# boqian-li/GarmentDreamer

Hardware: AMD Instinct MI355X
Metric: SDS iters/sec (rasterize+UNet+bwd), 100k Gaussians ×8 views @512², 1/2/4/8 GPU (higher is better)
Workload: dtype bf16

## Files before the change

garmentdreamer_amd/csrc/nn_conv3x3.hip:

```cpp
#include <hip/hip_runtime.h>
#include <stdlib.h>
#include <stdint.h>
#include <stdio.h>

#include <mutex>
#include <vector>

#include "../../include/gd_nn.h"
#include "nn_device.h"
#include "nn_host.h"

#ifndef GD_CONV_ABLATE
#define GD_CONV_ABLATE 0
#endif

namespace {

using namespace gdnn;

#ifndef GD_PATCH_EPI
#define GD_PATCH_EPI 0
#endif
typedef __attribute__((ext_vector_type(4))) float f32x4;

constexpr int BK = 64;

struct ConvGeom {
    int Hin, Win, Hg, Wg, sy, sx, Hout, Wout, osy, osx, ooy, oox, ntaps, back;
    int wtaps;
    uint64_t ty4, tx4, w4;
};

template <int BN, int BM, int WN, int WM>
__device__ __forceinline__ void conv3x3_nhwc_bf16_body(
    const uint16_t* __restrict__ in, const uint16_t* __restrict__ wt, const uint16_t* __restrict__ bias,
    int bias_img_stride, const uint16_t* __restrict__ residual, uint16_t* __restrict__ out, int Nimg, const ConvGeom& g,
    int Cin, int Cout, int tiles_n, int nwg, float* __restrict__ partial, int steps_per_split, int bid_raw, int split_idx)
{
    constexpr int THREADS = 64 * WN * WM;
    constexpr int NA = BM * 8 / THREADS;
    constexpr int NB = BN * 8 / THREADS;
    constexpr int FA = BN / WN / 32;
    constexpr int FB = BM / WM / 32;
    constexpr int kStage = (BM + BN) * BK * 2;
    extern __shared__ __attribute__((aligned(16))) char smem[];
    const int tid = threadIdx.x, lane = tid & 63;
    const int wave = __builtin_amdgcn_readfirstlane(tid >> 6);
    int bid = bid_raw;
    if ((nwg & 7) == 0) bid = (bid & 7) * (nwg >> 3) + (bid >> 3);
    const int tn = bid % tiles_n, tm = bid / tiles_n;
    const int m0 = tm * BM, n0 = tn * BN;
    const int HW = g.Hg * g.Wg;
    const int64_t M = (int64_t)Nimg * HW;
    const int H = g.Hin, W = g.Win;

    const uint32_t row_bytes = (uint32_t)Cin * 2u;
    const uint32_t back = (uint32_t)g.back * row_bytes;
    const __amdgpu_buffer_rsrc_t rs_in = buffer_rsrc((const char*)in - back, (uint32_t)Nimg * (uint32_t)(H * W) * row_bytes + back);
    const __amdgpu_buffer_rsrc_t rs_w = buffer_rsrc(wt, (uint32_t)Cout * (uint32_t)g.wtaps * row_bytes);

    uint32_t a_off[NA];
    int a_y[NA], a_x[NA];
    uint32_t b_off[NB];
#pragma unroll
    for (int i = 0; i < NA; i++) {
        const int q = tid + THREADS * i;
        const int line = q >> 4, c = (q & 15) ^ (line & 15);
        const int r = 2 * line + (c >> 3);
        const int64_t m = (int64_t)m0 + r;
        if (m < M) {
            const int nimg = (int)(m / HW);
            const int rem = (int)(m - (int64_t)nimg * HW);
            const int ga = rem / g.Wg;
            a_y[i] = ga * g.sy;
            a_x[i] = (rem - ga * g.Wg) * g.sx;
            a_off[i] = (uint32_t)((nimg * H + a_y[i]) * W + a_x[i]) * row_bytes + (uint32_t)(c & 7) * 16u;
        } else {
            a_y[i] = -100000; a_x[i] = 0; a_off[i] = kOOB;
        }
    }
#pragma unroll
    for (int i = 0; i < NB; i++) {
        const int q = tid + THREADS * i;
        const int line = q >> 4, c = (q & 15) ^ (line & 15);
        const int r = 2 * line + (c >> 3);
        const int co = n0 + r;
        b_off[i] = co < Cout ? (uint32_t)co * (uint32_t)g.wtaps * row_bytes + (uint32_t)(c & 7) * 16u : kOOB;
    }
    const int kc = Cin / BK;
    const int step0 = partial ? split_idx * steps_per_split : 0;
    const int step1 = partial ? min(g.ntaps * kc, step0 + steps_per_split) : g.ntaps * kc;
    const int nsteps = step1 - step0;
    const int tap0 = step0 / kc;

    int ld_tap = tap0, ld_c = step0 - tap0 * kc;
    uint32_t a_voff[NA];
    auto set_tap = [&](int tap) {
        const int dy = (int)((g.ty4 >> (4 * tap)) & 15u) - 8, dx = (int)((g.tx4 >> (4 * tap)) & 15u) - 8;
#pragma unroll
        for (int i = 0; i < NA; i++) {
            const int yy = a_y[i] + dy, xx = a_x[i] + dx;
            const bool ok = (unsigned)yy < (unsigned)H && (unsigned)xx < (unsigned)W;
            a_voff[i] = ok ? a_off[i] : kOOB;
        }
    };
    set_tap(tap0);
    auto issue = [&](int buf) {
        char* sA = smem + buf * kStage;
        char* sB = sA + BM * BK * 2;
        const int dy = (int)((g.ty4 >> (4 * ld_tap)) & 15u) - 8, dx = (int)((g.tx4 >> (4 * ld_tap)) & 15u) - 8;
        const uint32_t soff_a = (uint32_t)(dy * W + dx + g.back) * row_bytes + (uint32_t)ld_c * (BK * 2);
        const uint32_t soff_b = (uint32_t)((g.w4 >> (4 * ld_tap)) & 15u) * row_bytes + (uint32_t)ld_c * (BK * 2);
#if GD_CONV_ABLATE != 1 && GD_CONV_ABLATE != 2 && GD_CONV_ABLATE < 6
#pragma unroll
        for (int i = 0; i < NA; i++) bload_lds16(rs_in, a_voff[i], soff_a, sA + (wave * 64 + THREADS * i) * 16);
#endif
#if GD_CONV_ABLATE != 2 && GD_CONV_ABLATE < 6
#pragma unroll
        for (int i = 0; i < NB; i++) bload_lds16(rs_w, b_off[i], soff_b, sB + (wave * 64 + THREADS * i) * 16);
#endif
        if (++ld_c == kc) {
            ld_c = 0;
            if (++ld_tap < g.ntaps) set_tap(ld_tap);
        }
    };

    f32x16 acc[FA][FB];
#pragma unroll
    for (int a = 0; a < FA; a++)
#pragma unroll
        for (int b = 0; b < FB; b++)
#pragma unroll
            for (int k = 0; k < 16; k++) acc[a][b][k] = 0.f;

    const int wc = wave % WN, wp = wave / WN;
    const int frow = lane & 31, fk = lane >> 5;
    uint32_t w_rd[FA], p_rd[FB];
#pragma unroll
    for (int a = 0; a < FA; a++) w_rd[a] = (uint32_t)(BM * BK * 2 + swz(wc * (BN / WN) + a * 32 + frow, fk));
#pragma unroll
    for (int b = 0; b < FB; b++) p_rd[b] = (uint32_t)swz(wp * (BM / WM) + b * 32 + frow, fk);

#if GD_CONV_ABLATE == 4 || GD_CONV_ABLATE >= 6
    bf16x8_t wf0[FA], pf0[FB];
#pragma unroll
    for (int a = 0; a < FA; a++) wf0[a] = *(const bf16x8_t*)(smem + w_rd[a]);
#pragma unroll
    for (int b = 0; b < FB; b++) pf0[b] = *(const bf16x8_t*)(smem + p_rd[b]);
#endif
    issue(0);
#if GD_CONV_ABLATE == 8
    for (int s = 0; s < (nsteps > 1 ? 1 : nsteps); s++) {
#else
    for (int s = 0; s < nsteps; s++) {
#endif
        const int buf = s & 1;
        asm volatile("s_waitcnt vmcnt(0)" ::: "memory");
#if GD_CONV_ABLATE != 5 && GD_CONV_ABLATE != 6
        __syncthreads();
#endif
        if (s + 1 < nsteps) issue(buf ^ 1);
        const char* st = smem + buf * kStage;
#pragma unroll
        for (int kk = 0; kk < 4; kk++) {
            bf16x8_t wf[FA], pf[FB];
#if GD_CONV_ABLATE == 4 || GD_CONV_ABLATE >= 6
            if (s > 0) {
#pragma unroll
                for (int a = 0; a < FA; a++)
#pragma unroll
                    for (int b = 0; b < FB; b++)
                        acc[a][b] = __builtin_amdgcn_mfma_f32_32x32x16_bf16(wf0[a], pf0[b], acc[a][b], 0, 0, 0);
                continue;
            }
#endif
#pragma unroll
            for (int a = 0; a < FA; a++) wf[a] = *(const bf16x8_t*)(st + (w_rd[a] ^ (uint32_t)(kk << 5)));
#pragma unroll
            for (int b = 0; b < FB; b++) pf[b] = *(const bf16x8_t*)(st + (p_rd[b] ^ (uint32_t)(kk << 5)));
#pragma unroll
            for (int a = 0; a < FA; a++)
#pragma unroll
                for (int b = 0; b < FB; b++)
#if GD_CONV_ABLATE == 3
                    if (a == 0 && b == 0) acc[a][b] = __builtin_amdgcn_mfma_f32_32x32x16_bf16(wf[a], pf[b], acc[a][b], 0, 0, 0);
                    else { acc[a][b][0] += __builtin_bit_cast(float, (int)wf[a][0] ^ (int)pf[b][1]); }
#else
                    acc[a][b] = __builtin_amdgcn_mfma_f32_32x32x16_bf16(wf[a], pf[b], acc[a][b], 0, 0, 0);
#endif
        }
    }

#pragma unroll
    for (int b = 0; b < FB; b++) {
        const int64_t m = (int64_t)m0 + wp * (BM / WM) + b * 32 + (lane & 31);
        if (m >= M) continue;
        const int nimg = (int)(m / HW);
// ... 4 lines not shown
#pragma unroll
        for (int a = 0; a < FA; a++) {
#pragma unroll
            for (int q = 0; q < 4; q++) {
                const int co = n0 + wc * (BN / WN) + a * 32 + 8 * q + 4 * fk;
                if (co >= Cout) continue;
                float v[4];
#pragma unroll
                for (int e = 0; e < 4; e++) v[e] = acc[a][b][4 * q + e];
                if (partial) {
                    *(float4*)(partial + (((size_t)split_idx * nwg + bid) * (BN * BM / 4) +
                                          (((wave * FB + b) * FA + a) * 4 + q) * 64 + lane) * 4) = make_float4(v[0], v[1], v[2], v[3]);
                    continue;
                }
                if (bias_n) {
                    const uint2 bb = *(const uint2*)(bias_n + co);
                    v[0] += bf2f((uint16_t)(bb.x & 0xffff)); v[1] += bf2f((uint16_t)(bb.x >> 16));
                    v[2] += bf2f((uint16_t)(bb.y & 0xffff)); v[3] += bf2f((uint16_t)(bb.y >> 16));
                }
                if (residual) {
                    const uint2 rr = *(const uint2*)(residual + opix * Cout + co);
                    v[0] += bf2f((uint16_t)(rr.x & 0xffff)); v[1] += bf2f((uint16_t)(rr.x >> 16));
                    v[2] += bf2f((uint16_t)(rr.y & 0xffff)); v[3] += bf2f((uint16_t)(rr.y >> 16));
                }
                uint2 o;
                o.x = pack_bf16(v[0], v[1]);
                o.y = pack_bf16(v[2], v[3]);
                *(uint2*)(out + opix * Cout + co) = o;
            }
        }
    }
}

template <int BN, int BM, int WN, int WM>
__global__ __launch_bounds__(64 * WN * WM) void conv3x3_nhwc_bf16_kernel(
    const uint16_t* __restrict__ in, const uint16_t* __restrict__ wt, const uint16_t* __restrict__ bias,
    int bias_img_stride, const uint16_t* __restrict__ residual, uint16_t* __restrict__ out, int Nimg, const ConvGeom g,
    int Cin, int Cout, int tiles_n, int nwg, float* __restrict__ partial, int steps_per_split)
{
    conv3x3_nhwc_bf16_body<BN, BM, WN, WM>(in, wt, bias, bias_img_stride, residual, out, Nimg, g, Cin, Cout, tiles_n, nwg,
                                           partial, steps_per_split, (int)blockIdx.x, (int)blockIdx.y);
}

struct ConvGeomSet {
    ConvGeom g[4];
    const uint16_t* wt[4];
    int nwg[4];
    int n;
};

template <int BN, int BM, int WN, int WM>
__global__ __launch_bounds__(64 * WN * WM) void conv3x3_nhwc_bf16_multi_kernel(
    const uint16_t* __restrict__ in, const uint16_t* __restrict__ bias, int bias_img_stride,
    const uint16_t* __restrict__ residual, uint16_t* __restrict__ out, int Nimg, const ConvGeomSet gs, int Cin, int Cout,
    int tiles_n)
{
    const int cls = (int)blockIdx.z;
    const int nwg = gs.nwg[cls];
    if ((int)blockIdx.x >= nwg) return;
    conv3x3_nhwc_bf16_body<BN, BM, WN, WM>(in, gs.wt[cls], bias, bias_img_stride, residual, out, Nimg, gs.g[cls], Cin, Cout,
                                           tiles_n, nwg, nullptr, 0, (int)blockIdx.x, 0);
}

constexpr int kPatch = 18, kPatchPix = kPatch * kPatch;

__device__ __forceinline__ float silu_fast(float z) { return z * __builtin_amdgcn_rcpf(1.0f + __expf(-z)); }

__device__ __forceinline__ float row16_sum(float v)
{
    v += __builtin_bit_cast(float, __builtin_amdgcn_update_dpp(0, __builtin_bit_cast(int, v), 0xB1, 0xf, 0xf, false));
    v += __builtin_bit_cast(float, __builtin_amdgcn_update_dpp(0, __builtin_bit_cast(int, v), 0x4E, 0xf, 0xf, false));
    v += __builtin_bit_cast(float, __builtin_amdgcn_update_dpp(0, __builtin_bit_cast(int, v), 0x141, 0xf, 0xf, false));
    v += __builtin_bit_cast(float, __builtin_amdgcn_update_dpp(0, __builtin_bit_cast(int, v), 0x140, 0xf, 0xf, false));
    return v;
}

__device__ __forceinline__ void stat_accumulate(float2& st, uint2 o)
{
    const float r0 = __uint_as_float(o.x << 16), r1 = __uint_as_float(o.x & 0xffff0000u);
    const float r2 = __uint_as_float(o.y << 16), r3 = __uint_as_float(o.y & 0xffff0000u);
    st.x += (r0 + r1) + (r2 + r3);
    st.y += fmaf(r0, r0, fmaf(r1, r1, fmaf(r2, r2, r3 * r3)));
}

__device__ __forceinline__ void patch_col(int fn, int& rr, int& fx)
{
    if (fn < 4) { rr = 0; fx = fn; }
    else if (fn < 12) { rr = 1; fx = fn - 4; }
    else if (fn < 16) { rr = 0; fx = fn - 8; }
    else if (fn < 20) { rr = 1; fx = fn - 8; }
    else if (fn < 28) { rr = 0; fx = fn - 12; }
    else { rr = 1; fx = fn - 16; }
}
// ... 733 lines not shown
            }
        }
        if (stat_part) {
            const int rows = nwaves * 2, row = wave_g * 2 + ((lane >> 4) & 1);
#pragma unroll
            for (int a = 0; a < FA; a++) {
#pragma unroll
                for (int q = 0; q < 4; q++) {
                    const float sx = row16_sum(st[a][q].x), sy = row16_sum(st[a][q].y);
                    const int quad = 8 * a + 2 * q + fk;
                    if ((lane & 15) == 0)
                        *(float2*)(stat_part + (((size_t)n * (Cout >> 2) + quad) * rows + row) * 2) = make_float2(sx, sy);
                }
            }
        }
    }
}

__global__ void conv3x3_flip_weights_kernel(const uint16_t* __restrict__ w, uint16_t* __restrict__ wf, int Cout,
                                            int Cin)
{
    const size_t total = (size_t)Cout * 9 * Cin;
    for (size_t i = (size_t)blockIdx.x * blockDim.x + threadIdx.x; i < total; i += (size_t)gridDim.x * blockDim.x) {
        const int co = (int)(i % Cout);
        const int tap = (int)((i / Cout) % 9);
        const int ci = (int)(i / ((size_t)Cout * 9));
        wf[i] = w[((size_t)co * 9 + (8 - tap)) * Cin + ci];
    }
}

int g_route_scale = 1;
int g_force_split = -1;
int g_force_variant = -1;

struct ConvEnv {
    int split_px = 0;
    int multi_class = 1;
    int patch_persistent = 1;
    int first_grid = 2048;
};
const ConvEnv& conv_env()
{
    static const ConvEnv env = [] {
        ConvEnv v;
        if (const char* e = getenv("GD_NN_SPLIT_PX")) v.split_px = atoi(e);
        if (const char* e = getenv("GD_NN_CONV_MULTI")) v.multi_class = atoi(e);
        if (const char* e = getenv("GD_NN_PATCH_PERSISTENT")) v.patch_persistent = atoi(e) != 0;
        if (const char* e = getenv("GD_NN_FIRST_GRID")) v.first_grid = atoi(e) > 0 ? atoi(e) : v.first_grid;
        return v;
    }();
    return env;
}

int num_cus(int dev)
{
    static const int cus = [dev] {
        int c = 0;
        return hipDeviceGetAttribute(&c, hipDeviceAttributeMultiprocessorCount, dev) == hipSuccess && c > 0 ? c : 256;
    }();
    return cus;
}

struct ConvProf {
    std::mutex mu;
    bool on = false;
    struct Rec { hipEvent_t a, b; };
// ... 168 lines not shown
    if (!x || !weight || !y) return fail(GD_NN_ERR_INVALID_ARG, "null pointer");
    if (N <= 0 || H <= 0 || W <= 0 || Cin % BK || Cout % 4 || Cin <= 0 || Cout <= 0)
        return fail(GD_NN_ERR_INVALID_ARG, "conv3x3: need Cin % 64 == 0 and Cout % 4 == 0");
    g = ConvGeom{};
    g.Hin = g.Hg = g.Hout = H;
    g.Win = g.Wg = g.Wout = W;
    g.sy = g.sx = g.osy = g.osx = 1;
    for (int ky = 0; ky < 3; ky++)
        for (int kx = 0; kx < 3; kx++) add_tap(g, ky - 1, kx - 1, ky * 3 + kx);
    return GD_NN_OK;
}

static int launch_conv(hipStream_t s, const void* x, const void* weight, const void* bias, int bias_img_stride,
                       const void* residual, void* y, int N, ConvGeom g, int Cin, int Cout, void* ws = nullptr,
                       size_t ws_bytes = 0)
{
    const int dev = current_device();
    if (dev < 0) return dev;
    if (const int r = finalize_geom(g, N, Cin, Cout)) return r;
    const int64_t M = (int64_t)N * g.Hg * g.Wg;
    if (M <= 0) return GD_NN_OK;
    int split = ws ? choose_split(M, Cout, g.ntaps, Cin) : 1;
    if (split > 1 && ws_bytes < split_ws_bytes(split, M, Cout)) split = 1;
    float* partial = split > 1 ? (float*)ws : nullptr;
    const int total_steps = g.ntaps * (Cin / BK);
    const int tps = split > 1 ? (total_steps + split - 1) / split : total_steps;
    if (split > 1) split = (total_steps + tps - 1) / tps;
    const int spx = split > 1 ? split_tile_px(M, Cout) : 128;
    int variant = split > 1 ? (spx == 256 ? 1 : 0) : g_force_variant;
    if (variant < 0 && small_tile_nosplit(M, Cout, g.ntaps, Cin)) variant = 6;
    if (variant < 0)
        variant = Cout <= 32 && M * g_route_scale >= (1 << 18) ? 4 : tile_variant(M, Cin, Cout);
    ProfScope prof(s);
#define GD_LAUNCH(BN_, BM_, WN_, WM_)                                                                              \
    do {                                                                                                           \
        constexpr auto kern = conv3x3_nhwc_bf16_kernel<BN_, BM_, WN_, WM_>;                                        \
        constexpr int lds = 2 * (BN_ + BM_) * BK * 2;                                                              \
        if (const int r = reserve_lds<kern>(dev, lds)) return r;                                                   \
        const int tiles_m = (int)((M + BM_ - 1) / BM_), tiles_n = (Cout + BN_ - 1) / BN_;                          \
        const int nwg = tiles_m * tiles_n;                                                                         \
        hipLaunchKernelGGL(kern, dim3(nwg, split), dim3(64 * WN_ * WM_), lds, s, (const uint16_t*)x,               \
                           (const uint16_t*)weight, (const uint16_t*)bias, bias_img_stride,                        \
                           (const uint16_t*)residual, (uint16_t*)y, N, g, Cin, Cout, tiles_n, nwg, partial, tps);  \
    } while (0)
    if (variant == 2) GD_LAUNCH(256, 256, 2, 4);
    else if (variant == 4) GD_LAUNCH(32, 256, 1, 4);
    else if (variant == 1) GD_LAUNCH(128, 256, 2, 4);
    else if (variant == 5) GD_LAUNCH(64, 128, 2, 2);
    else if (variant == 6) GD_LAUNCH(64, 64, 2, 2);
    else if (variant == 7) GD_LAUNCH(128, 64, 2, 2);
    else GD_LAUNCH(128, 128, 2, 2);
#undef GD_LAUNCH
    if (split > 1) {
        const int tiles_n = (Cout + 127) / 128, nwg = (int)((M + spx - 1) / spx) * tiles_n;
        if (spx == 256)
            hipLaunchKernelGGL(conv_splitk_reduce_kernel<256>, dim3((unsigned)nwg * 32u), dim3(256), 0, s, partial, split, nwg,
                               tiles_n, M, Cout, g.Hg * g.Wg, g.Wg, g.Hout, g.Wout, g.osy, g.osx, g.ooy, g.oox,
                               (const uint16_t*)bias, bias_img_stride, (const uint16_t*)residual, (uint16_t*)y);
        else
            hipLaunchKernelGGL(conv_splitk_reduce_kernel<128>, dim3((unsigned)nwg * 16u), dim3(256), 0, s, partial, split, nwg,
                               tiles_n, M, Cout, g.Hg * g.Wg, g.Wg, g.Hout, g.Wout, g.osy, g.osx, g.ooy, g.oox,
                               (const uint16_t*)bias, bias_img_stride, (const uint16_t*)residual, (uint16_t*)y);
    }
    prof.close(2.0 * (double)M * Cout * (double)g.ntaps * Cin,
               2.0 * ((double)N * g.Hin * g.Win * Cin + (double)g.ntaps * Cin * Cout + (double)M * Cout +
                      (residual ? (double)M * Cout : 0.0)));
    return launch_status();
}

static int launch_conv_multi(hipStream_t s, const void* x, const void* const* weights, const void* bias, int bias_img_stride,
                             const void* residual, void* y, int N, ConvGeom* geoms, int ncls, int Cin, int Cout, bool may_split)
{
    if (!conv_env().multi_class || ncls < 2 || ncls > 4 || g_force_variant >= 0 || g_force_split >= 0) return 0;
    const int dev = current_device();
    if (dev < 0) return dev;
    int64_t Msum = 0;
    double flops = 0, bytes = 0;
    for (int c = 0; c < ncls; c++) {
        ConvGeom& g = geoms[c];
        if (const int r = finalize_geom(g, N, Cin, Cout)) return r;
        const int64_t M = (int64_t)N * g.Hg * g.Wg;
        if (M <= 0) return 0;
        if (may_split && choose_split(M, Cout, g.ntaps, Cin) > 1) return 0;
        Msum += M;
        flops += 2.0 * (double)M * Cout * (double)g.ntaps * Cin;
        bytes += 2.0 * ((double)g.ntaps * Cin * Cout + (double)M * Cout + (residual ? (double)M * Cout : 0.0));
    }
    bytes += 2.0 * (double)N * geoms[0].Hin * geoms[0].Win * Cin;
    const int variant = tile_variant(Msum, Cin, Cout);
    ProfScope prof(s);
#define GD_LAUNCH_M(BN_, BM_, WN_, WM_)                                                                            \
    do {                                                                                                           \
        constexpr auto kern = conv3x3_nhwc_bf16_multi_kernel<BN_, BM_, WN_, WM_>;                                  \
        constexpr int lds = 2 * (BN_ + BM_) * BK * 2;                                                              \
        if (const int r = reserve_lds<kern>(dev, lds)) return r;                                                   \
        ConvGeomSet gs = {};                                                                                       \
        gs.n = ncls;                                                                                               \
        const int tiles_n = (Cout + BN_ - 1) / BN_;                                                                \
        int nmax = 0;                                                                                              \
        for (int c = 0; c < ncls; c++) {                                                                           \
            gs.g[c] = geoms[c];                                                                                    \
            gs.wt[c] = (const uint16_t*)weights[c];                                                                \
            const int64_t M = (int64_t)N * geoms[c].Hg * geoms[c].Wg;                                              \
            gs.nwg[c] = (int)((M + BM_ - 1) / BM_) * tiles_n;                                                      \
            nmax = gs.nwg[c] > nmax ? gs.nwg[c] : nmax;                                                            \
        }                                                                                                          \
        hipLaunchKernelGGL(kern, dim3(nmax, 1, ncls), dim3(64 * WN_ * WM_), lds, s, (const uint16_t*)x,            \
                           (const uint16_t*)bias, bias_img_stride, (const uint16_t*)residual, (uint16_t*)y, N, gs, \
                           Cin, Cout, tiles_n);                                                                    \
    } while (0)
    if (variant == 2) GD_LAUNCH_M(256, 256, 2, 4);
    else if (variant == 1) GD_LAUNCH_M(128, 256, 2, 4);
    else GD_LAUNCH_M(128, 128, 2, 2);
#undef GD_LAUNCH_M
    prof.close(flops, bytes);
    const int r = launch_status();
    return r < 0 ? r : 1;
}

static int launch_patch(void* stream, const void* x, const float* mean_rstd, const void* gamma, const void* beta,
                        int groups, int apply_silu, const void* weight, const void* bias, int bias_img_stride,
                        const void* residual, void* y, int N, int H, int W, int Cin, int Cout,
                        float* stat_part = nullptr)
{
    if (!x || !weight || !y) return fail(GD_NN_ERR_INVALID_ARG, "null pointer");
    if (N <= 0 || H <= 0 || W <= 0 || Cin % BK || Cout % 4 || Cin <= 0 || Cout <= 0)
        return fail(GD_NN_ERR_INVALID_ARG, "conv3x3_gn: need Cin % 64 == 0 and Cout % 4 == 0");
    if (mean_rstd && (!gamma || !beta || groups <= 0 || Cin % groups))
        return fail(GD_NN_ERR_INVALID_ARG, "conv3x3_gn: GroupNorm needs gamma, beta and Cin % groups == 0");
    if ((double)N * H * W * Cin * 2.0 >= 2147483648.0 || (double)Cout * 9.0 * Cin * 2.0 >= 2147483648.0)
        return fail(GD_NN_ERR_INVALID_ARG, "conv3x3_gn: activation / weight tensor must be < 2 GiB (32-bit buffer offsets)");
    const TiledArgs a = {stream, x, mean_rstd, gamma, beta, groups, apply_silu, weight, bias, bias_img_stride, residual, y,
                         N, H, W, Cin, Cout, stat_part};
    int bn = (Cout % 256 == 0) ? 256 : 128;
    if (g_force_variant == 1 || g_force_variant == 0) bn = 128;
    if (g_force_variant == 2) bn = 256;
    const bool persistent = conv_env().patch_persistent != 0;
    constexpr auto lds = [](int slab) { return 2 * (kPatchPix + 4) * BK * 2 + 2 * slab * BK * 2; };
    if (mean_rstd && bn == 256 && !gn_table_fits(lds(256), Cin)) bn = 128;
    if (bn == 256)
        return mean_rstd ? launch_tiled<conv3x3_gn_patch_kernel<256, 2, 4, true>>(a, lds(256), 16, 256, false)
                         : launch_tiled<conv3x3_patch_stream_kernel<256, 2, 4, false>>(a, lds(256), 16, 256, persistent);
    return mean_rstd ? launch_tiled<conv3x3_gn_patch_kernel<128, 2, 4, true>>(a, lds(128), 16, 128, false)
                     : launch_tiled<conv3x3_patch_stream_kernel<128, 2, 4, false>>(a, lds(128), 16, 128, persistent);
}

// ... 399 lines not shown
    {
        ConvGeom tmp[4] = {gs4[0], gs4[1], gs4[2], gs4[3]};
        const int r = launch_conv_multi((hipStream_t)stream, x, ws4, bias, 0, nullptr, y, N, tmp, 4, Cin, Cout, false);
        if (r != 0) return r < 0 ? r : GD_NN_OK;
    }
    for (int c = 0; c < 4; c++) {
        const int r = launch_conv((hipStream_t)stream, x, ws4[c], bias, 0, nullptr, y, N, gs4[c], Cin, Cout);
        if (r < 0) return r;
    }
    return GD_NN_OK;
}

int gd_nn_linear_forward(void* stream, const void* x, const void* weight, const void* bias, const void* residual, void* y,
                         int64_t M, int K, int Nout)
{
    if (!x || !weight || !y) return fail(GD_NN_ERR_INVALID_ARG, "null pointer");
    if (M <= 0 || M > 0x7fffffff || K <= 0 || K % BK || Nout <= 0 || Nout % 4)
        return fail(GD_NN_ERR_INVALID_ARG, "linear: need K % 64 == 0 and Nout % 4 == 0");
    ConvGeom g = {};
    g.Hin = g.Hg = g.Hout = 1;
    g.Win = g.Wg = g.Wout = (int)M;
    g.sy = g.sx = g.osy = g.osx = 1;
    g.wtaps = 1;
    add_tap(g, 0, 0, 0);
    return launch_conv((hipStream_t)stream, x, weight, bias, 0, residual, y, 1, g, K, Nout);
}

int gd_nn_conv_force_variant(int v)
{
    g_force_variant = v;
    return GD_NN_OK;
}

int gd_nn_conv_profile_enable(int on)
{
    std::lock_guard<std::mutex> lk(g_cprof.mu);
    g_cprof.on = on != 0;
    return GD_NN_OK;
}

int gd_nn_conv_profile_reset(void)
{
    std::lock_guard<std::mutex> lk(g_cprof.mu);
    g_cprof.total_ms = g_cprof.total_flops = g_cprof.total_bytes = 0;
    g_cprof.launches = 0;
    return GD_NN_OK;
}

int gd_nn_conv_profile_read(double* total_ms, int64_t* launches, double* total_flops)
{
    std::lock_guard<std::mutex> lk(g_cprof.mu);
    for (auto& r : g_cprof.pending) {
        float ms = 0.f;
        if (hipEventSynchronize(r.b) == hipSuccess && hipEventElapsedTime(&ms, r.a, r.b) == hipSuccess) {
            g_cprof.total_ms += ms;
            g_cprof.launches += 1;
        }
        g_cprof.pool.push_back(r.a);
        g_cprof.pool.push_back(r.b);
    }
    g_cprof.pending.clear();
    if (total_ms) *total_ms = g_cprof.total_ms;
    if (launches) *launches = g_cprof.launches;
    if (total_flops) *total_flops = g_cprof.total_flops;
    return GD_NN_OK;
}
// ... 44 lines not shown
```

garmentdreamer_amd/nn_ops.py:

```python
from __future__ import annotations

import ctypes as C
import os
import weakref

import torch
import torch.nn.functional as F

_HERE = os.path.dirname(os.path.abspath(__file__))
_LIB_PATH = os.path.join(_HERE, "libgd_nn.so")
_LIB_OVERRIDDEN = False
_lib = None


def use_library(path: str) -> None:
    global _LIB_PATH, _LIB_OVERRIDDEN
    if _lib is not None:
        raise RuntimeError("libgd_nn.so is already loaded")
    _LIB_PATH, _LIB_OVERRIDDEN = os.path.abspath(path), True


_vp, _i, _f = C.c_void_p, C.c_int, C.c_float
SIGNATURES = {
    "gd_nn_groupnorm_silu_forward": (_i, [_vp, _vp, _vp, _vp, _vp, _i, _i, _i, _i, _f, _i, _vp, _vp]),
# ... 16 lines not shown
    "gd_nn_groupnorm_stats": (_i, [_vp, _vp, _i, _i, _i, _i, _f, _vp, _vp]),
    "gd_nn_groupnorm_silu_forward_fp8": (_i, [_vp, _vp, _vp, _vp, _vp, _i, _i, _i, _i, _f, _i, _vp, _vp, _f]),
    "gd_nn_conv3x3_gn_forward": (_i, [_vp, _vp, _vp, _vp, _vp, _i, _i, _vp, _vp, _i, _vp, _vp, _i, _i, _i, _i, _i]),
    "gd_nn_linear_320_supported": (_i, [C.c_int64, _i, _i]),
    "gd_nn_linear_320_forward": (_i, [_vp, _vp, _vp, _vp, _vp, C.c_int64]),
    "gd_nn_linear_k320_forward": (_i, [_vp, _vp, _vp, _vp, _vp, C.c_int64, _i]),
    "gd_nn_linear_k320_geglu_forward": (_i, [_vp, _vp, _vp, _vp, _vp, C.c_int64, _i]),
    "gd_nn_linear_320_last_error": (C.c_char_p, []),
    "gd_nn_conv3x3_stat_rows": (C.c_size_t, [_i, _i, _i, _i, _i]),
    "gd_nn_conv3x3_first_stat_rows": (C.c_size_t, [_i, _i, _i, _i, _i]),
    "gd_nn_conv3x3_first_forward_stats": (_i, [_vp, _vp, _vp, _vp, _vp, _i, _i, _i, _i, _i, _vp]),
    "gd_nn_conv3x3_gn_forward_stats": (_i, [_vp, _vp, _vp, _vp, _vp, _i, _i, _vp, _vp, _i, _vp, _vp, _i, _i, _i, _i, _i,
                                            _vp]),
    "gd_nn_conv3x3_forward_stats": (_i, [_vp, _vp, _vp, _vp, _i, _vp, _vp, _i, _i, _i, _i, _i, _vp]),
    "gd_nn_conv3x3_wino_supported": (_i, [_i, _i, _i, _i, _i]),
    "gd_nn_conv3x3_wino_weights": (_i, [_vp, _vp, _vp, _i, _i]),
    "gd_nn_conv3x3_wino_weights_bytes": (C.c_size_t, [_i, _i]),
    "gd_nn_conv3x3_wino_forward": (_i, [_vp, _vp, _vp, _vp, _i, _vp, _vp, _i, _i, _i, _i, _i, _vp]),
    "gd_nn_conv3x3_wino_gn_forward": (_i, [_vp, _vp, _vp, _vp, _vp, _i, _i, _vp, _vp, _i, _vp, _vp, _i, _i, _i, _i, _i, _vp]),
    "gd_nn_conv3x3_wide_supported": (_i, [_i, _i, _i, _i, _i]),
    "gd_nn_conv3x3_wide_weights": (_i, [_vp, _vp, _vp, _i, _i]),
    "gd_nn_conv3x3_wide_weights_bytes": (C.c_size_t, [_i, _i]),
    "gd_nn_conv3x3_wide_forward": (_i, [_vp, _vp, _vp, _vp, _i, _vp, _vp, _i, _i, _i, _i, _i, _vp]),
    "gd_nn_conv3x3_wide_gn_forward": (_i, [_vp, _vp, _vp, _vp, _vp, _i, _i, _vp, _vp, _i, _vp, _vp, _i, _i, _i, _i, _i, _vp]),
    "gd_nn_groupnorm_finish_partials": (_i, [_vp, _vp, _i, C.c_size_t, _i, _i, _i, _f, _vp]),
    "gd_nn_conv3x3_first_forward": (_i, [_vp, _vp, _vp, _vp, _vp, _i, _i, _i, _i, _i]),
    "gd_nn_conv3x3_s2_forward": (_i, [_vp, _vp, _vp, _vp, _vp, _i, _i, _i, _i, _i, _i]),
    "gd_nn_conv3x3_s2_dgrad": (_i, [_vp, _vp, _vp, _vp, _i, _i, _i, _i, _i, _i]),
    "gd_nn_conv3x3_s2_ws_bytes": (C.c_size_t, [_i, _i, _i, _i, _i, _i, _i]),
    "gd_nn_conv3x3_s2_forward_ws": (_i, [_vp, _vp, _vp, _vp, _vp, _i, _i, _i, _i, _i, _i, _vp, C.c_size_t]),
    "gd_nn_conv3x3_s2_dgrad_ws": (_i, [_vp, _vp, _vp, _vp, _i, _i, _i, _i, _i, _i, _vp, C.c_size_t]),
    "gd_nn_conv3x3_up2_forward": (_i, [_vp, _vp, _vp, _vp, _vp, _vp, _i, _i, _i, _i, _i]),
    "gd_nn_conv_force_variant": (_i, [_i]),
    "gd_nn_linear_forward": (_i, [_vp, _vp, _vp, _vp, _vp, _vp, C.c_int64, _i, _i]),
    "gd_nn_gemm_supported": (_i, [C.c_int64, _i, _i, _i]),
    "gd_nn_gemm_forward": (_i, [_vp, _vp, _vp, _vp, _vp, _vp, C.c_int64, _i, _i]),
    "gd_nn_gemm_geglu_forward": (_i, [_vp, _vp, _vp, _vp, _vp, C.c_int64, _i, _i]),
    "gd_nn_gemm_last_error": (C.c_char_p, []),
    "gd_nn_conv_profile_enable": (_i, [_i]),
    "gd_nn_conv_profile_reset": (_i, []),
    "gd_nn_conv_profile_read": (_i, [C.POINTER(C.c_double), C.POINTER(C.c_int64), C.POINTER(C.c_double)]),
    "gd_nn_conv_profile_read_bytes": (_i, [C.POINTER(C.c_double)]),
    "gd_nn_geglu_forward": (_i, [_vp, _vp, _vp, C.c_int64, _i]),
    "gd_nn_geglu_backward": (_i, [_vp, _vp, _vp, _vp, C.c_int64, _i]),
    "gd_nn_conv1x1_c8": (_i, [_vp, _vp, _vp, _vp, _vp, C.c_int64, _i]),
    "gd_nn_softmax_rows_forward": (_i, [_vp, _vp, _vp, C.c_int64, _i]),
    "gd_nn_softmax_rows_backward": (_i, [_vp, _vp, _vp, _vp, C.c_int64, _i]),
    "gd_nn_layernorm_backward": (_i, [_vp, _vp, _vp, _vp, _vp, _vp, C.c_int64, _i, C.c_float]),
    "gd_nn_add_layernorm_forward": (_i, [_vp, _vp, _vp, _vp, _vp, _f, _vp, _vp, C.c_int64, _i]),
    "gd_nn_add_layernorm_forward_bcast": (_i, [_vp, _vp, _vp, _vp, _vp, _f, _vp, _vp, C.c_int64, _i, C.c_int64]),
    "gd_nn_join_stat_rows": (C.c_size_t, [_i, _i, _i]),
    "gd_nn_add_gn_partials": (_i, [_vp, _vp, _vp, _vp, _vp, _i, _i, _i, _i]),
    "gd_nn_concat_gn_partials": (_i, [_vp, _vp, _vp, _vp, _vp, _i, _i, _i, _i, _i]),
    "gd_nn_attention_ws_bytes": (C.c_size_t, [_i, _i, _i]),
    "gd_nn_attention_d64_forward": (_i, [_vp, _vp, _vp, _vp, _vp, _vp, _i, _i, _i, _i, C.c_int64, _i, C.c_int64, _i,
                                         C.c_int64, _i, C.c_int64, _i, _f, _i]),
    "gd_nn_attention_d64_forward_lse": (_i, [_vp, _vp, _vp, _vp, _vp, _vp, _vp, _i, _i, _i, _i, C.c_int64, _i, C.c_int64, _i,
                                             C.c_int64, _i, C.c_int64, _i, _f, _i]),
    "gd_nn_attention_bwd_ws_bytes": (C.c_size_t, [_i, _i, _i, _i]),
    "gd_nn_attention_d64_backward": (_i, [_vp] * 11 + [_i, _i, _i, _i] + [C.c_int64, _i] * 8 + [_f, _i]),
    "gd_nn_attention_d64_forward_vt": (_i, [_vp, _vp, _vp, _vp, _vp, _i, _i, _i, _i, C.c_int64, _i, C.c_int64, _i, C.c_int64, _i,
                                            _f]),
    "gd_nn_attention_d64_forward_vt_strided": (_i, [_vp, _vp, _vp, _vp, _vp, _i, _i, _i, _i, C.c_int64, _i, C.c_int64, _i, C.c_int64,
                                                    C.c_int64, _i, _f, _i]),
    "gd_nn_attention_last_error": (C.c_char_p, []),
    "gd_nn_vae_prologue_forward": (_i, [_vp, _vp, _vp, _i, _i, _i, _i, _i]),
# ... 1951 lines not shown
```

include/gd_nn.h:

```cpp
#ifndef GD_NN_H_INCLUDED
#define GD_NN_H_INCLUDED

#include <stddef.h>
#include <stdint.h>

#ifdef __cplusplus
extern "C" {
#endif

#define GD_NN_OK 0
#define GD_NN_ERR_INVALID_ARG (-1)
#define GD_NN_ERR_HIP (-2)

int gd_nn_groupnorm_silu_forward(void* stream, const void* x, void* y, const void* gamma, const void* beta, int N,
                                 int HW, int C, int G, float eps, int apply_silu, double* stats_ws,
                                 float* mean_rstd);

int gd_nn_groupnorm_silu_backward(void* stream, const void* x, const void* dy, const void* gamma,
                                  const void* beta, const float* mean_rstd, void* dx, int N, int HW, int C, int G,
                                  int apply_silu, double* stats_ws, float* group_sums ,
                                  const void* add);

size_t gd_nn_groupnorm_ws_bytes(int N, int G);

int gd_nn_conv3x3_forward(void* stream, const void* x, const void* weight, const void* bias, int bias_img_stride,
                          const void* residual, void* y, int N, int H, int W, int Cin, int Cout);

int gd_nn_conv3x3_flip_weights(void* stream, const void* weight, void* flipped, int Cout, int Cin);

int gd_nn_conv3x3_first_dgrad_supported(int N, int H, int W, int Cin, int Cout);
int gd_nn_conv3x3_first_dgrad_weights(void* stream, const void* weight, void* wpack, int Cout, int Cin);
int gd_nn_conv3x3_first_dgrad(void* stream, const void* dy, const void* wpack, void* dx4, int N, int H, int W, int Cin, int Cout);

int gd_nn_conv_force_variant(int v);

int gd_nn_linear_forward(void* stream, const void* x, const void* weight, const void* bias, const void* residual, void* y,
                         int64_t M, int K, int Nout);
int gd_nn_gemm_supported(int64_t M, int K, int N, int geglu);
int gd_nn_gemm_forward(void* stream, const void* x, const void* weight, const void* bias, const void* residual, void* y,
                       int64_t M, int K, int N);
int gd_nn_gemm_geglu_forward(void* stream, const void* x, const void* weight, const void* bias, void* y, int64_t M, int K,
                             int inner);
const char* gd_nn_gemm_last_error(void);
int gd_nn_conv_profile_enable(int on);
int gd_nn_conv_profile_reset(void);
int gd_nn_conv_profile_read(double* total_ms, int64_t* launches, double* total_flops);
int gd_nn_conv_profile_read_bytes(double* total_bytes);

size_t gd_nn_conv3x3_ws_bytes(int N, int H, int W, int Cin, int Cout);
int gd_nn_conv3x3_forward_ws(void* stream, const void* x, const void* weight, const void* bias, int bias_img_stride,
                             const void* residual, void* y, int N, int H, int W, int Cin, int Cout, void* ws,
                             size_t ws_bytes);
int gd_nn_conv_force_split(int s);
int gd_nn_conv_set_route_scale(int k);

int gd_nn_groupnorm_silu_fused_supported(int N, int HW, int C, int G);
int gd_nn_groupnorm_silu_fused_forward(void* stream, const void* x, void* y, const void* gamma, const void* beta, int N,
                                       int HW, int C, int G, float eps, int apply_silu);
int gd_nn_groupnorm_silu_fused_forward_stats(void* stream, const void* x, void* y, const void* gamma, const void* beta, int N,
                                             int HW, int C, int G, float eps, int apply_silu, float* mean_rstd);
int gd_nn_groupnorm_silu_fused_backward_supported(int N, int HW, int C, int G);
int gd_nn_groupnorm_silu_fused_backward(void* stream, const void* x, const void* dy, const void* gamma, const void* beta,
                                        const float* mean_rstd, void* dx, int N, int HW, int C, int G, int apply_silu);

int gd_nn_groupnorm_stats(void* stream, const void* x, int N, int HW, int C, int G, float eps, double* stats_ws,
                          float* mean_rstd);

// ... 155 lines not shown
```

Baseline: 23.84.

## Add multi-stage LDS ring pipeline with selectable stage depth and channel width to conv3x3

Generalizes the conv3x3 implicit-GEMM kernel from a fixed double buffer of 64-channel stages to a D-deep ring of 32- or 64-channel stages. It waits on partial vmcnt counts so several loads stay in flight, and adjusts launch bounds for occupancy. Default scheduling stays on the old 2x64 path, except the multi-class 128x256 short-K case, which now uses 3 stages of 32 channels. It also adds an API to force other schedules for tuning. The deeper ring is meant to hide global-load latency at the cost of more LDS and smaller per-stage MFMA work.

```diff
diff --git a/garmentdreamer_amd/csrc/nn_conv3x3.hip b/garmentdreamer_amd/csrc/nn_conv3x3.hip
--- a/garmentdreamer_amd/csrc/nn_conv3x3.hip
+++ b/garmentdreamer_amd/csrc/nn_conv3x3.hip
@@ -31,18 +31,57 @@
     uint64_t ty4, tx4, w4;
 };
 
-template <int BN, int BM, int WN, int WM>
+template <int SC>
+struct IgemmStage {
+    static_assert(SC == 64 || SC == 32, "stage of 64 or 32 channels");
+    static constexpr int kChunks = SC / 8;
+    static constexpr int kRows = 16 / kChunks;
+    static constexpr int kMask = SC == 64 ? 15 : 3;
+    static __device__ __forceinline__ int off(int row, int j)
+    {
+        const int line = row / kRows;
+        return line * 256 + ((((row % kRows) * kChunks) | j) ^ (line & kMask)) * 16;
+    }
+};
+
+constexpr int igemm_lds(int BN, int BM, int D, int SC) { return D * (BN + BM) * SC * 2; }
+constexpr int igemm_wgs(int BN, int BM, int D, int SC) { return 2 * igemm_lds(BN, BM, D, SC) <= 160 * 1024 ? 2 : 1; }
+
+template <int N>
+__device__ __forceinline__ void igemm_wait_barrier()
+{
+    static_assert(N >= 0 && N <= 63, "vmcnt is a 6-bit counter");
+    asm volatile("s_waitcnt vmcnt(%0) lgkmcnt(0)" ::"n"(N) : "memory");
+    __builtin_amdgcn_s_barrier();
+    asm volatile("" ::: "memory");
+}
+template <int L, int K>
+__device__ __forceinline__ void igemm_ring_wait(int k)
+{
+    if constexpr (K == 0) {
+        igemm_wait_barrier<0>();
+    } else {
+        if (k >= K) igemm_wait_barrier<K * L>();
+        else igemm_ring_wait<L, K - 1>(k);
+    }
+}
+
+template <int BN, int BM, int WN, int WM, int D, int SC>
 __device__ __forceinline__ void conv3x3_nhwc_bf16_body(
     const uint16_t* __restrict__ in, const uint16_t* __restrict__ wt, const uint16_t* __restrict__ bias,
     int bias_img_stride, const uint16_t* __restrict__ residual, uint16_t* __restrict__ out, int Nimg, const ConvGeom& g,
     int Cin, int Cout, int tiles_n, int nwg, float* __restrict__ partial, int steps_per_split, int bid_raw, int split_idx)
 {
+    using Stage = IgemmStage<SC>;
     constexpr int THREADS = 64 * WN * WM;
-    constexpr int NA = BM * 8 / THREADS;
-    constexpr int NB = BN * 8 / THREADS;
+    constexpr int NA = BM * Stage::kChunks / THREADS;
+    constexpr int NB = BN * Stage::kChunks / THREADS;
+    static_assert(NA >= 1 && NB >= 1 && NA * THREADS == BM * Stage::kChunks && NB * THREADS == BN * Stage::kChunks,
+                  "every thread moves whole chunks of both tiles");
+    static_assert(D >= 2 && (D - 2) * (NA + NB) <= 63, "ring depth against the vmcnt counter");
     constexpr int FA = BN / WN / 32;
     constexpr int FB = BM / WM / 32;
-    constexpr int kStage = (BM + BN) * BK * 2;
+    constexpr int kStage = (BM + BN) * SC * 2;
     extern __shared__ __attribute__((aligned(16))) char smem[];
     const int tid = threadIdx.x, lane = tid & 63;
     const int wave = __builtin_amdgcn_readfirstlane(tid >> 6);
@@ -65,8 +104,8 @@
 #pragma unroll
     for (int i = 0; i < NA; i++) {
         const int q = tid + THREADS * i;
-        const int line = q >> 4, c = (q & 15) ^ (line & 15);
-        const int r = 2 * line + (c >> 3);
+        const int line = q >> 4, c = (q & 15) ^ (line & Stage::kMask);
+        const int r = Stage::kRows * line + c / Stage::kChunks;
         const int64_t m = (int64_t)m0 + r;
         if (m < M) {
             const int nimg = (int)(m / HW);
@@ -74,7 +113,7 @@
             const int ga = rem / g.Wg;
             a_y[i] = ga * g.sy;
             a_x[i] = (rem - ga * g.Wg) * g.sx;
-            a_off[i] = (uint32_t)((nimg * H + a_y[i]) * W + a_x[i]) * row_bytes + (uint32_t)(c & 7) * 16u;
+            a_off[i] = (uint32_t)((nimg * H + a_y[i]) * W + a_x[i]) * row_bytes + (uint32_t)(c % Stage::kChunks) * 16u;
         } else {
             a_y[i] = -100000; a_x[i] = 0; a_off[i] = kOOB;
         }
@@ -82,14 +121,14 @@
 #pragma unroll
     for (int i = 0; i < NB; i++) {
         const int q = tid + THREADS * i;
-        const int line = q >> 4, c = (q & 15) ^ (line & 15);
-        const int r = 2 * line + (c >> 3);
+        const int line = q >> 4, c = (q & 15) ^ (line & Stage::kMask);
+        const int r = Stage::kRows * line + c / Stage::kChunks;
         const int co = n0 + r;
-        b_off[i] = co < Cout ? (uint32_t)co * (uint32_t)g.wtaps * row_bytes + (uint32_t)(c & 7) * 16u : kOOB;
-    }
-    const int kc = Cin / BK;
-    const int step0 = partial ? split_idx * steps_per_split : 0;
-    const int step1 = partial ? min(g.ntaps * kc, step0 + steps_per_split) : g.ntaps * kc;
+        b_off[i] = co < Cout ? (uint32_t)co * (uint32_t)g.wtaps * row_bytes + (uint32_t)(c % Stage::kChunks) * 16u : kOOB;
+    }
+    const int kc = Cin / SC;
+    const int step0 = partial ? split_idx * steps_per_split * (BK / SC) : 0;
+    const int step1 = partial ? min(g.ntaps * kc, step0 + steps_per_split * (BK / SC)) : g.ntaps * kc;
     const int nsteps = step1 - step0;
     const int tap0 = step0 / kc;
 
@@ -107,10 +146,10 @@
     set_tap(tap0);
     auto issue = [&](int buf) {
         char* sA = smem + buf * kStage;
-        char* sB = sA + BM * BK * 2;
+        char* sB = sA + BM * SC * 2;
         const int dy = (int)((g.ty4 >> (4 * ld_tap)) & 15u) - 8, dx = (int)((g.tx4 >> (4 * ld_tap)) & 15u) - 8;
-        const uint32_t soff_a = (uint32_t)(dy * W + dx + g.back) * row_bytes + (uint32_t)ld_c * (BK * 2);
-        const uint32_t soff_b = (uint32_t)((g.w4 >> (4 * ld_tap)) & 15u) * row_bytes + (uint32_t)ld_c * (BK * 2);
+        const uint32_t soff_a = (uint32_t)(dy * W + dx + g.back) * row_bytes + (uint32_t)ld_c * (SC * 2);
+        const uint32_t soff_b = (uint32_t)((g.w4 >> (4 * ld_tap)) & 15u) * row_bytes + (uint32_t)ld_c * (SC * 2);
 #if GD_CONV_ABLATE != 1 && GD_CONV_ABLATE != 2 && GD_CONV_ABLATE < 6
 #pragma unroll
         for (int i = 0; i < NA; i++) bload_lds16(rs_in, a_voff[i], soff_a, sA + (wave * 64 + THREADS * i) * 16);
@@ -137,9 +176,9 @@
     const int frow = lane & 31, fk = lane >> 5;
     uint32_t w_rd[FA], p_rd[FB];
 #pragma unroll
-    for (int a = 0; a < FA; a++) w_rd[a] = (uint32_t)(BM * BK * 2 + swz(wc * (BN / WN) + a * 32 + frow, fk));
-#pragma unroll
-    for (int b = 0; b < FB; b++) p_rd[b] = (uint32_t)swz(wp * (BM / WM) + b * 32 + frow, fk);
+    for (int a = 0; a < FA; a++) w_rd[a] = (uint32_t)(BM * SC * 2 + Stage::off(wc * (BN / WN) + a * 32 + frow, fk));
+#pragma unroll
+    for (int b = 0; b < FB; b++) p_rd[b] = (uint32_t)Stage::off(wp * (BM / WM) + b * 32 + frow, fk);
 
 #if GD_CONV_ABLATE == 4 || GD_CONV_ABLATE >= 6
     bf16x8_t wf0[FA], pf0[FB];
@@ -148,21 +187,26 @@
 #pragma unroll
     for (int b = 0; b < FB; b++) pf0[b] = *(const bf16x8_t*)(smem + p_rd[b]);
 #endif
-    issue(0);
+    int wr = 0;
+#pragma unroll
+    for (int p = 0; p < D - 1; p++)
+        if (p < nsteps) { issue(wr); wr = wr + 1 == D ? 0 : wr + 1; }
+    int buf = 0;
 #if GD_CONV_ABLATE == 8
     for (int s = 0; s < (nsteps > 1 ? 1 : nsteps); s++) {
 #else
     for (int s = 0; s < nsteps; s++) {
 #endif
-        const int buf = s & 1;
+#if GD_CONV_ABLATE != 5 && GD_CONV_ABLATE != 6
+        igemm_ring_wait<NA + NB, D - 2>(nsteps - 1 - s);
+#else
         asm volatile("s_waitcnt vmcnt(0)" ::: "memory");
-#if GD_CONV_ABLATE != 5 && GD_CONV_ABLATE != 6
-        __syncthreads();
 #endif
-        if (s + 1 < nsteps) issue(buf ^ 1);
+        if (s + D - 1 < nsteps) { issue(wr); wr = wr + 1 == D ? 0 : wr + 1; }
         const char* st = smem + buf * kStage;
-#pragma unroll
-        for (int kk = 0; kk < 4; kk++) {
+        buf = buf + 1 == D ? 0 : buf + 1;
+#pragma unroll
+        for (int kk = 0; kk < SC / 16; kk++) {
             bf16x8_t wf[FA], pf[FB];
 #if GD_CONV_ABLATE == 4 || GD_CONV_ABLATE >= 6
             if (s > 0) {
@@ -233,13 +277,13 @@
     }
 }
 
-template <int BN, int BM, int WN, int WM>
-__global__ __launch_bounds__(64 * WN * WM) void conv3x3_nhwc_bf16_kernel(
+template <int BN, int BM, int WN, int WM, int D, int SC>
+__global__ __launch_bounds__(64 * WN * WM, igemm_wgs(BN, BM, D, SC) * WN * WM / 4) void conv3x3_nhwc_bf16_kernel(
     const uint16_t* __restrict__ in, const uint16_t* __restrict__ wt, const uint16_t* __restrict__ bias,
     int bias_img_stride, const uint16_t* __restrict__ residual, uint16_t* __restrict__ out, int Nimg, const ConvGeom g,
     int Cin, int Cout, int tiles_n, int nwg, float* __restrict__ partial, int steps_per_split)
 {
-    conv3x3_nhwc_bf16_body<BN, BM, WN, WM>(in, wt, bias, bias_img_stride, residual, out, Nimg, g, Cin, Cout, tiles_n, nwg,
+    conv3x3_nhwc_bf16_body<BN, BM, WN, WM, D, SC>(in, wt, bias, bias_img_stride, residual, out, Nimg, g, Cin, Cout, tiles_n, nwg,
                                            partial, steps_per_split, (int)blockIdx.x, (int)blockIdx.y);
 }
 
@@ -250,8 +294,8 @@
     int n;
 };
 
-template <int BN, int BM, int WN, int WM>
-__global__ __launch_bounds__(64 * WN * WM) void conv3x3_nhwc_bf16_multi_kernel(
+template <int BN, int BM, int WN, int WM, int D, int SC>
+__global__ __launch_bounds__(64 * WN * WM, igemm_wgs(BN, BM, D, SC) * WN * WM / 4) void conv3x3_nhwc_bf16_multi_kernel(
     const uint16_t* __restrict__ in, const uint16_t* __restrict__ bias, int bias_img_stride,
     const uint16_t* __restrict__ residual, uint16_t* __restrict__ out, int Nimg, const ConvGeomSet gs, int Cin, int Cout,
     int tiles_n)
@@ -259,7 +303,7 @@
     const int cls = (int)blockIdx.z;
     const int nwg = gs.nwg[cls];
     if ((int)blockIdx.x >= nwg) return;
-    conv3x3_nhwc_bf16_body<BN, BM, WN, WM>(in, gs.wt[cls], bias, bias_img_stride, residual, out, Nimg, gs.g[cls], Cin, Cout,
+    conv3x3_nhwc_bf16_body<BN, BM, WN, WM, D, SC>(in, gs.wt[cls], bias, bias_img_stride, residual, out, Nimg, gs.g[cls], Cin, Cout,
                                            tiles_n, nwg, nullptr, 0, (int)blockIdx.x, 0);
 }
 
@@ -1059,6 +1103,23 @@
 int g_route_scale = 1;
 int g_force_split = -1;
 int g_force_variant = -1;
+int g_igemm_stages = 0;
+int g_igemm_channels = 0;
+
+constexpr int kSchedOld = 264;
+constexpr int kSched128x128[] = {kSchedOld, 432, 532};
+constexpr int kSched128x256[] = {kSchedOld, 332, 632, 364};
+constexpr int kSched256x256[] = {kSchedOld, 432, 532};
+constexpr int kSchedShortK = 332;
+inline bool igemm_multi_short_k(int max_taps, int Cin) { return max_taps * (Cin / BK) <= 8; }
+template <int N>
+int igemm_schedule(const int (&built)[N], int dflt = kSchedOld)
+{
+    const int forced = g_igemm_stages * 100 + g_igemm_channels;
+    for (int i = 0; i < N; i++)
+        if (built[i] == forced) return forced;
+    return dflt;
+}
 
 struct ConvEnv {
     int split_px = 0;
@@ -1293,10 +1354,10 @@
     if (variant < 0)
         variant = Cout <= 32 && M * g_route_scale >= (1 << 18) ? 4 : tile_variant(M, Cin, Cout);
     ProfScope prof(s);
-#define GD_LAUNCH(BN_, BM_, WN_, WM_)                                                                              \
+#define GD_LAUNCH(BN_, BM_, WN_, WM_, D_, SC_)                                                                     \
     do {                                                                                                           \
-        constexpr auto kern = conv3x3_nhwc_bf16_kernel<BN_, BM_, WN_, WM_>;                                        \
-        constexpr int lds = 2 * (BN_ + BM_) * BK * 2;                                                              \
+        constexpr auto kern = conv3x3_nhwc_bf16_kernel<BN_, BM_, WN_, WM_, D_, SC_>;                               \
+        constexpr int lds = igemm_lds(BN_, BM_, D_, SC_);                                                          \
         if (const int r = reserve_lds<kern>(dev, lds)) return r;                                                   \
         const int tiles_m = (int)((M + BM_ - 1) / BM_), tiles_n = (Cout + BN_ - 1) / BN_;                          \
         const int nwg = tiles_m * tiles_n;                                                                         \
@@ -1304,13 +1365,27 @@
                            (const uint16_t*)weight, (const uint16_t*)bias, bias_img_stride,                        \
                            (const uint16_t*)residual, (uint16_t*)y, N, g, Cin, Cout, tiles_n, nwg, partial, tps);  \
     } while (0)
-    if (variant == 2) GD_LAUNCH(256, 256, 2, 4);
-    else if (variant == 4) GD_LAUNCH(32, 256, 1, 4);
-    else if (variant == 1) GD_LAUNCH(128, 256, 2, 4);
-    else if (variant == 5) GD_LAUNCH(64, 128, 2, 2);
-    else if (variant == 6) GD_LAUNCH(64, 64, 2, 2);
-    else if (variant == 7) GD_LAUNCH(128, 64, 2, 2);
-    else GD_LAUNCH(128, 128, 2, 2);
+    if (variant == 2) {
+        const int sch = igemm_schedule(kSched256x256);
+        if (sch == 432) GD_LAUNCH(256, 256, 2, 4, 4, 32);
+        else if (sch == 532) GD_LAUNCH(256, 256, 2, 4, 5, 32);
+        else GD_LAUNCH(256, 256, 2, 4, 2, 64);
+    } else if (variant == 1) {
+        const int sch = igemm_schedule(kSched128x256);
+        if (sch == 332) GD_LAUNCH(128, 256, 2, 4, 3, 32);
+        else if (sch == 632) GD_LAUNCH(128, 256, 2, 4, 6, 32);
+        else if (sch == 364) GD_LAUNCH(128, 256, 2, 4, 3, 64);
+        else GD_LAUNCH(128, 256, 2, 4, 2, 64);
+    } else if (variant == 4) GD_LAUNCH(32, 256, 1, 4, 2, 64);
+    else if (variant == 5) GD_LAUNCH(64, 128, 2, 2, 2, 64);
+    else if (variant == 6) GD_LAUNCH(64, 64, 2, 2, 2, 64);
+    else if (variant == 7) GD_LAUNCH(128, 64, 2, 2, 2, 64);
+    else {
+        const int sch = igemm_schedule(kSched128x128);
+        if (sch == 432) GD_LAUNCH(128, 128, 2, 2, 4, 32);
+        else if (sch == 532) GD_LAUNCH(128, 128, 2, 2, 5, 32);
+        else GD_LAUNCH(128, 128, 2, 2, 2, 64);
+    }
 #undef GD_LAUNCH
     if (split > 1) {
         const int tiles_n = (Cout + 127) / 128, nwg = (int)((M + spx - 1) / spx) * tiles_n;
@@ -1350,10 +1425,10 @@
     bytes += 2.0 * (double)N * geoms[0].Hin * geoms[0].Win * Cin;
     const int variant = tile_variant(Msum, Cin, Cout);
     ProfScope prof(s);
-#define GD_LAUNCH_M(BN_, BM_, WN_, WM_)                                                                            \
+#define GD_LAUNCH_M(BN_, BM_, WN_, WM_, D_, SC_)                                                                   \
     do {                                                                                                           \
-        constexpr auto kern = conv3x3_nhwc_bf16_multi_kernel<BN_, BM_, WN_, WM_>;                                  \
-        constexpr int lds = 2 * (BN_ + BM_) * BK * 2;                                                              \
+        constexpr auto kern = conv3x3_nhwc_bf16_multi_kernel<BN_, BM_, WN_, WM_, D_, SC_>;                         \
+        constexpr int lds = igemm_lds(BN_, BM_, D_, SC_);                                                          \
         if (const int r = reserve_lds<kern>(dev, lds)) return r;                                                   \
         ConvGeomSet gs = {};                                                                                       \
         gs.n = ncls;                                                                                               \
@@ -1370,9 +1445,25 @@
                            (const uint16_t*)bias, bias_img_stride, (const uint16_t*)residual, (uint16_t*)y, N, gs, \
                            Cin, Cout, tiles_n);                                                                    \
     } while (0)
-    if (variant == 2) GD_LAUNCH_M(256, 256, 2, 4);
-    else if (variant == 1) GD_LAUNCH_M(128, 256, 2, 4);
-    else GD_LAUNCH_M(128, 128, 2, 2);
+    if (variant == 2) {
+        const int sch = igemm_schedule(kSched256x256);
+        if (sch == 432) GD_LAUNCH_M(256, 256, 2, 4, 4, 32);
+        else if (sch == 532) GD_LAUNCH_M(256, 256, 2, 4, 5, 32);
+        else GD_LAUNCH_M(256, 256, 2, 4, 2, 64);
+    } else if (variant == 1) {
+        int max_taps = 0;
+        for (int c = 0; c < ncls; c++) max_taps = geoms[c].ntaps > max_taps ? geoms[c].ntaps : max_taps;
+        const int sch = igemm_schedule(kSched128x256, igemm_multi_short_k(max_taps, Cin) ? kSchedShortK : kSchedOld);
+        if (sch == 332) GD_LAUNCH_M(128, 256, 2, 4, 3, 32);
+        else if (sch == 632) GD_LAUNCH_M(128, 256, 2, 4, 6, 32);
+        else if (sch == 364) GD_LAUNCH_M(128, 256, 2, 4, 3, 64);
+        else GD_LAUNCH_M(128, 256, 2, 4, 2, 64);
+    } else {
+        const int sch = igemm_schedule(kSched128x128);
+        if (sch == 432) GD_LAUNCH_M(128, 128, 2, 2, 4, 32);
+        else if (sch == 532) GD_LAUNCH_M(128, 128, 2, 2, 5, 32);
+        else GD_LAUNCH_M(128, 128, 2, 2, 2, 64);
+    }
 #undef GD_LAUNCH_M
     prof.close(flops, bytes);
     const int r = launch_status();
@@ -1838,6 +1929,19 @@
     return GD_NN_OK;
 }
 
+int gd_nn_conv_igemm_schedule(int stages, int stage_channels)
+{
+    const int sch = stages * 100 + stage_channels;
+    bool built = sch == 0;
+    for (const int b : kSched128x128) built |= b == sch;
+    for (const int b : kSched128x256) built |= b == sch;
+    for (const int b : kSched256x256) built |= b == sch;
+    if (!built) return fail(GD_NN_ERR_INVALID_ARG, "conv igemm schedule: no tile is built with this (stages, stage_channels)");
+    g_igemm_stages = stages;
+    g_igemm_channels = stage_channels;
+    return GD_NN_OK;
+}
+
 int gd_nn_conv_profile_enable(int on)
 {
     std::lock_guard<std::mutex> lk(g_cprof.mu);
diff --git a/garmentdreamer_amd/nn_ops.py b/garmentdreamer_amd/nn_ops.py
--- a/garmentdreamer_amd/nn_ops.py
+++ b/garmentdreamer_amd/nn_ops.py
@@ -72,6 +72,7 @@
     "gd_nn_conv3x3_s2_dgrad_ws": (_i, [_vp, _vp, _vp, _vp, _i, _i, _i, _i, _i, _i, _vp, C.c_size_t]),
     "gd_nn_conv3x3_up2_forward": (_i, [_vp, _vp, _vp, _vp, _vp, _vp, _i, _i, _i, _i, _i]),
     "gd_nn_conv_force_variant": (_i, [_i]),
+    "gd_nn_conv_igemm_schedule": (_i, [_i, _i]),
     "gd_nn_linear_forward": (_i, [_vp, _vp, _vp, _vp, _vp, _vp, C.c_int64, _i, _i]),
     "gd_nn_gemm_supported": (_i, [C.c_int64, _i, _i, _i]),
     "gd_nn_gemm_forward": (_i, [_vp, _vp, _vp, _vp, _vp, _vp, C.c_int64, _i, _i]),
diff --git a/include/gd_nn.h b/include/gd_nn.h
--- a/include/gd_nn.h
+++ b/include/gd_nn.h
@@ -33,6 +33,7 @@
 int gd_nn_conv3x3_first_dgrad(void* stream, const void* dy, const void* wpack, void* dx4, int N, int H, int W, int Cin, int Cout);
 
 int gd_nn_conv_force_variant(int v);
+int gd_nn_conv_igemm_schedule(int stages, int stage_channels);
 
 int gd_nn_linear_forward(void* stream, const void* x, const void* weight, const void* bias, const void* residual, void* y,
                          int64_t M, int K, int Nout);
```

New measurement: 23.84 (median of 2 runs). No clear change (+0.0%).
